# T-amairi/block-lanczos-algorithm-parallelization

Hardware: AMD Instinct MI355X
Metric: nnz*n mod-p MAC/s (higher is better)
Workload: dtype u64; 1 GPU; JGD_GL7d/GL7d19-shape synthetic: 1911130x1955309, 37322725 nnz, --prime 2^61-1 --n 8 --left; parallelism=single GPU, matrix=seeded synthetic, uniform columns (SURVEY 8(d)); real .mtx not on the box, timing=one region of 2050 steps, max over ranks per region

## Files before the change

### block-lanczos-algorithm-parallelization_amd/csrc/blz_api.hip

```cpp
#include <dlfcn.h>
#include <unistd.h>
#include <rccl/rccl.h>

#include <algorithm>
#include <cmath>
#include <cstdio>
#include <cstdlib>
#include <cstring>
#include <memory>
#include <vector>
#include <atomic>
#include <chrono>
#include <condition_variable>
#include <mutex>

#include "blz_internal.h"
#include "blz_kernels.h"
#include "blz_border.h"
#include "blz_devio.h"
#include "blz_devalg.h"
#include "blz_devsmall.h"
#include "blz_devfuse.h"
#include "blz_devrank.h"
#include "blz_devw32.h"
// ... 144 lines not shown
	u64 *small = nullptr, *partial = nullptr;
	u64 *dot_send = nullptr;
	u64 *dot_recv = nullptr;
	int max_dot_blocks = 0;
	DevCtl *ctl = nullptr;
	DevCtl host_ctl{};
	DevCtl *ctl_pinned = nullptr, *ctl_pinned_dev = nullptr;
	ncclComm_t comm = nullptr;
	blz_loop_group *loop = nullptr;
	int loop_rank = -1;
	std::vector<int32_t> perm[2], inv[2];
	bool reorder = true;
	bool pack = true;
	bool fuse_dot = true;
	bool selfdot = true;
	u64 *partial_self = nullptr;
	int max_self_blocks = 0;
	bool fuse_local_off = false;
	int un = 0;
	bool use_graph = false;
	bool explicit_p = false;
	bool p_implicit = false;
	long long rot_swaps = 0;
	hipGraphExec_t iter_graph = nullptr;
	bool external_exchange = false;
	bool force_comm = false;
	hipStream_t cstream = nullptr;
	hipEvent_t ev_snap_go = nullptr, ev_snap_done = nullptr;
	void *snap_host[2] = { nullptr, nullptr };
	void *snap_dev[2] = { nullptr, nullptr };
// ... 201 lines not shown
		c->cfg.mfma_img = nullptr;
		HIPCHK(hipMalloc(&c->cfg.mfma_img, ortho_mfma_image_bytes()));
	}
	{
		const char *npn = getenv("BLZ_NO_PANEL");
		c->cfg.panel = !(npn && npn[0] == '1');
	}
	const char *np = getenv("BLZ_NO_PACK");
	c->pack = !(np && np[0] == '1');
	const char *nr = getenv("BLZ_NO_REORDER");
	c->reorder = !(nr && nr[0] == '1');
	const char *nf = getenv("BLZ_NO_FUSE");
	c->fuse_dot = !(nf && nf[0] == '1');
	const char *nsf = getenv("BLZ_NO_SELFDOT");
	c->selfdot = !(nsf && nsf[0] == '1');
	const char *ug = getenv("BLZ_GRAPH");
	c->use_graph = ug && ug[0] == '1';
	const char *xp = getenv("BLZ_EXPLICIT_P");
	c->explicit_p = xp && xp[0] == '1';
	if (const char *ac = getenv("BLZ_AG_CHUNKS"))
		if (atoi(ac) >= 1 && atoi(ac) <= 64)
			c->ag_chunks = atoi(ac);
	HIPCHK(hipStreamCreateWithFlags(&c->stream, hipStreamNonBlocking));
	HIPCHK(hipStreamCreateWithFlags(&c->xstream, hipStreamNonBlocking));
	HIPCHK(hipEventCreateWithFlags(&c->ev_prod, hipEventDisableTiming));
	HIPCHK(hipEventCreate(&c->ev0));
	HIPCHK(hipEventCreate(&c->ev1));
	HIPCHK(hipMalloc(&c->small, small_words(np_) * sizeof(u64)));
	HIPCHK(hipMemset(c->small, 0, small_words(np_) * sizeof(u64)));
	{
		int rc_ = explicit_p_state(c);
		if (rc_ != BLZ_OK)
			return rc_;
	}
	HIPCHK(hipMalloc(&c->dot_send, (size_t)2 * np_ * np_ * sizeof(u64)));
	HIPCHK(hipMemset(c->dot_send, 0, (size_t)2 * np_ * np_ * sizeof(u64)));
	HIPCHK(hipMalloc(&c->dot_recv, (size_t)2 * np_ * np_ * sizeof(u64)));
	HIPCHK(hipMemset(c->dot_recv, 0, (size_t)2 * np_ * np_ * sizeof(u64)));
	c->max_dot_blocks = c->cfg.num_cu * (np_ <= 8 ? 16 : 8);
	HIPCHK(hipMalloc(&c->partial, (size_t)c->max_dot_blocks * 2 * np_ * np_ * sizeof(u64)));
	if (c->selfdot && np_ <= 8) {
		c->max_self_blocks = c->cfg.num_cu * std::max(8, c->cfg.spmv_blocks_per_cu) + 8;
		HIPCHK(hipMalloc(&c->partial_self, (size_t)c->max_self_blocks * np_ * np_ * sizeof(u64)));
	}
// ... 972 lines not shown
static inline bool iteration_fuses(const blz_ctx *c)
{
	return c->fuse_dot && !c->fuse_local_off && spmv_dot_supported(c->cfg) && c->count[0] > 0 && !c->short_side[c->right];
}

static inline bool selfdot_path(const blz_ctx *c)
{
	if (!c->selfdot || !c->partial_self || !c->have_matrix || !iteration_fuses(c) || exchanging(c) || c->nranks != 1 || c->bd.rhs
	    || c->use_graph || c->short_side[0] || c->short_side[1] || c->csr[0].size() != 1 || c->csr[1].size() != 1)
		return false;
	return spmv_self_ok(c->cfg, c->csr[!c->right][0], false, c->max_self_blocks)
	       && spmv_self_ok(c->cfg, c->csr[c->right][0], true, c->max_dot_blocks);
}

extern "C" int blz_selfdot_active(const blz_ctx *c) { return c && selfdot_path(c) ? 1 : 0; }

static void plan_launch(const SpmvGrids &g, blz_plan_launch *o)
{
	o->form = g.form == SPMV_FORM_PANEL ? BLZ_FORM_PANEL : (g.form == SPMV_FORM_STAGED ? BLZ_FORM_STAGED : BLZ_FORM_SPMV);
	o->xcd_ranges = g.xcd;
	o->split_log2 = g.split_log2;
	o->st_gathers = g.gathers;
	o->grid_stream = g.blocks;
	o->grid_heavy = g.hb;
	o->grid_combine = g.cb;
	o->grid_medium = g.mb;
}

extern "C" int blz_slab_plan(const blz_ctx *c, int transpose, int piece, blz_plan *out)
{
// ... 247 lines not shown
	int g = 0;
	while (g + 1 < c->nranks && c->bounds[sd][g + 1] <= r)
		g++;
	return g;
}

static int small_off(const blz_ctx *c, int which, int *words)
{
	const int nn = c->cfg.n * c->cfg.n;
	*words = which == BLZ_D ? c->cfg.n : nn;
	switch (which) {
	case BLZ_VTAV: return 0;
	case BLZ_VTAAV: return nn;
	case BLZ_WINV: return 2 * nn;
	case BLZ_D: return 3 * nn;
	default: return -1;
	}
}

extern "C" int blz_set_small(blz_ctx *c, int which, const uint64_t *host)
{
	if (!c || !host)
		return blz_fail(BLZ_EINVAL, "blz_set_small: NULL argument");
	HIPCHK(hipSetDevice(c->device));
	int words, off = small_off(c, which, &words);
	if (off < 0)
		return blz_fail(BLZ_EINVAL, "blz_set_small: unknown operand %d", which);
	HIPCHK(hipStreamSynchronize(c->stream));
	std::vector<u64> dev((size_t)words, 0);
	const int un = c->un, np = c->cfg.n;
// ... 352 lines not shown
{
	NEED_MATRIX(c);
	int rc = materialize_p(c);
	if (rc != BLZ_OK)
		return rc;
	rc = enqueue_ortho(c);
	if (rc != BLZ_OK)
		return rc;
	HIPCHK(hipStreamSynchronize(c->stream));
	return BLZ_OK;
}

static int enqueue_iteration(blz_ctx *c)
{
	int rc;
	if (selfdot_path(c)) {
		int nb1 = 0, nb2 = 0;
		{
			Span sp(c, PK_SPMV1);
			HIPCHK(launch_spmv_self(c->cfg, c->csr[!c->right][0], operand_ptr(c, BLZ_V), slab_ptr(c, BLZ_TMP), false,
						c->partial_self, c->max_self_blocks, &nb1, c->ctl, c->stream));
		}
		{
			Span sp(c, PK_SPMV2);
			HIPCHK(launch_spmv_self(c->cfg, c->csr[c->right][0], operand_ptr(c, BLZ_TMP), slab_ptr(c, BLZ_AV), true, c->partial,
						c->max_dot_blocks, &nb2, c->ctl, c->stream));
		}
		{
			Span sp(c, PK_DOT);
			HIPCHK(launch_dot_finalize_pair(c->cfg, c->partial_self, nb1, c->partial, nb2, c->small, c->ctl, c->stream));
		}
	} else if ((rc = enqueue_product(c, !c->right, BLZ_V, BLZ_TMP, false, nullptr)) != BLZ_OK) {
		return rc;
	} else if (iteration_fuses(c)) {
		int nb = 0;
		if ((rc = enqueue_product(c, c->right, BLZ_TMP, BLZ_AV, true, &nb)) != BLZ_OK) return rc;
		{
			Span sp(c, PK_DOT);
			HIPCHK(launch_dot_finalize(c->cfg, c->partial, nb, dot_out(c), c->ctl, c->stream));
		}
		if ((rc = allreduce_dots(c)) != BLZ_OK) return rc;
	} else {
		if ((rc = enqueue_product(c, c->right, BLZ_TMP, BLZ_AV, false, nullptr)) != BLZ_OK) return rc;
		if ((rc = enqueue_dot(c)) != BLZ_OK) return rc;
	}
	const bool img = ortho_uses_mfma(c->cfg, c->count[0]);
	const bool rot = img && !c->use_graph && !c->explicit_p;
	{
		Span sp(c, PK_SEMI);
		HIPCHK(launch_semi_inverse(c->cfg, dot_sums(c), c->small, c->ctl, 1, img, c->stream, rot ? c->un : 0));
	}
	if (!rot)
		return enqueue_ortho(c, img);
	const int np = c->cfg.n;
	Span sp(c, PK_ORTHO);
	if (np == 16)
		HIPCHK(launch_block_mul_gated(c->cfg, c->slab[BLZ_P], c->count[0], np, np, c->small + small_Emat(np), c->ctl,
					      c->small + small_materialize(np), c->stream));
	HIPCHK(launch_orthogonalize_rotate(c->cfg, slab_ptr(c, BLZ_V), slab_ptr(c, BLZ_AV), slab_ptr(c, BLZ_P), c->count[0],
					   c->small, c->ctl, c->stream));
	std::swap(c->slab[BLZ_V], c->slab[BLZ_P]);
	c->p_implicit = true;
	c->rot_swaps++;
	return BLZ_OK;
}
// ... 1981 lines not shown
```

### block-lanczos-algorithm-parallelization_amd/csrc/blz_kernels.h

```cpp
#ifndef BLZ_KERNELS_H
#define BLZ_KERNELS_H

#include <hip/hip_runtime.h>
#include <type_traits>
#include "modp.h"

#define HEAVY_SEG 4096u
struct HeavySeg {
	int row;
	u32 k0, k1;
	int whole_row;
};
struct HeavyRow {
	int row, first, count;
};

struct XcdRows {
	long long begin[9];
};

struct DevCsr {
	int64_t rows = 0, cols = 0, nnz = 0;
	u32 *row_ptr = nullptr;
	int *col_idx = nullptr;
// ... 80 lines not shown
SpmvGrids spmv_grids(const KernelCfg &c, const DevCsr &A, bool dot, int max_blocks);

hipError_t launch_spmv(const KernelCfg &c, const DevCsr &A, const void *X, void *Y, int accum, const DevCtl *ctl,
		       hipStream_t s);

bool spmv_dot_supported(const KernelCfg &c);
hipError_t launch_spmv_dot(const KernelCfg &c, const DevCsr &A, const void *X, void *Y, const void *Vd, int accum,
			   u64 *partial, int max_blocks, int *nblocks, const DevCtl *ctl, hipStream_t s);

hipError_t launch_block_dot(const KernelCfg &c, const void *V, const void *AV, int64_t rows, u64 *partial,
			    int max_blocks, int *nblocks, const DevCtl *ctl, hipStream_t s);
hipError_t launch_dot_finalize(const KernelCfg &c, const u64 *partial, int nblocks, u64 *out, const DevCtl *ctl,
			       hipStream_t s);

bool spmv_self_ok(const KernelCfg &c, const DevCsr &A, bool second, int max_blocks);
hipError_t launch_spmv_self(const KernelCfg &c, const DevCsr &A, const void *X, void *Y, bool second, u64 *partial,
			    int max_blocks, int *nblocks, const DevCtl *ctl, hipStream_t s);
hipError_t launch_dot_finalize_pair(const KernelCfg &c, const u64 *pa, int na, const u64 *pb, int nb, u64 *out, const DevCtl *ctl,
				    hipStream_t s);
hipError_t launch_dot_finalize_half(const KernelCfg &c, const u64 *partial, int nblocks, u64 *out, int half, const DevCtl *ctl,
				    hipStream_t s);

hipError_t launch_semi_inverse(const KernelCfg &c, const u64 *sums, u64 *small, DevCtl *ctl, int in_loop, int build_img,
			       hipStream_t s, int rot_un = 0);

hipError_t launch_orthogonalize(const KernelCfg &c, void *V, const void *AV, void *P, int64_t rows,
				const u64 *small, const DevCtl *ctl, hipStream_t s, bool img_ready = false);
bool ortho_uses_mfma(const KernelCfg &c, int64_t rows);

hipError_t launch_publish_ctl(const DevCtl *ctl, DevCtl *host_mapped, hipStream_t s);

hipError_t launch_copy(const KernelCfg &c, void *dst, const void *src, size_t bytes, hipStream_t s);

hipError_t launch_reduce_modp(const KernelCfg &c, void *dst, const void *src, int64_t words, const DevCtl *ctl, hipStream_t s);

size_t ortho_mfma_image_bytes(void);
bool ortho_mfma_supported(const KernelCfg &c);
hipError_t launch_orthogonalize_mfma(const KernelCfg &c, void *V, const void *AV, void *P, int64_t rows, const u64 *small,
				     const DevCtl *ctl, hipStream_t s, bool img_ready, bool rotate = false);
// ... 11 lines not shown

int rref_partial_blocks(const KernelCfg &c, int64_t rows, int n);
hipError_t launch_rref_partial(const KernelCfg &c, const void *X, int64_t rows, int ld, int n, u64 *stack, int *ctl,
			       hipStream_t s);
hipError_t launch_rref_merge(const KernelCfg &c, const u64 *stack, int64_t rows, const int *rows_dev, int n, u64 *E, int *info,
			     hipStream_t s);
hipError_t launch_block_mul(const KernelCfg &c, void *X, int64_t rows, int ld, int n, const u64 *Z, hipStream_t s);
hipError_t launch_block_mul_gated(const KernelCfg &c, void *X, int64_t rows, int ld, int n, const u64 *Z, const DevCtl *ctl,
				  const u64 *gate, hipStream_t s);

__host__ __device__ constexpr size_t small_E(int n) { return (size_t)6 * n * n; }
__host__ __device__ constexpr size_t small_Emat(int n) { return (size_t)7 * n * n; }
__host__ __device__ constexpr size_t small_skip_p(int n) { return (size_t)8 * n * n; }
__host__ __device__ constexpr size_t small_materialize(int n) { return (size_t)8 * n * n + 1; }
__host__ __device__ constexpr size_t small_words(int n) { return (size_t)8 * n * n + 8; }

#ifdef __cplusplus
template <typename T> struct TypeTag { using type = T; };
template <int V> using IntTag = std::integral_constant<int, V>;
template <bool V> using BoolTag = std::integral_constant<bool, V>;
#define DISPATCH_INLINE static inline __attribute__((always_inline))

template <typename F> DISPATCH_INLINE auto with_word_reducer(const KernelCfg &c, F &&f)
{
	if (c.word == 4)
		return c.mers == 31 ? f(TypeTag<u32>{}, IntTag<31>{}) : f(TypeTag<u32>{}, IntTag<0>{});
	return c.mers == 61 ? f(TypeTag<u64>{}, IntTag<61>{}) : f(TypeTag<u64>{}, IntTag<0>{});
}

template <int... Gs, typename F> DISPATCH_INLINE bool with_lane_group(int G, F &&f)
// ... 35 lines not shown
```

### block-lanczos-algorithm-parallelization_amd/csrc/blz_kernels.hip

```cpp
#include "blz_kernels.h"
#include "ortho_img.h"

#include <algorithm>
#include <atomic>
#include <type_traits>

#define BLOCK 256

MODP_DEV u64 shfl64(u64 x, int src)
{
	const u32 lo = (u32)__shfl((int)(u32)x, src, 64), hi = (u32)__shfl((int)(u32)(x >> 32), src, 64);
	return ((u64)hi << 32) | lo;
}

MODP_DEV u64 bperm64(u64 x, int src_lane_x4)
{
	const u32 lo = (u32)__builtin_amdgcn_ds_bpermute(src_lane_x4, (int)(u32)x);
	const u32 hi = (u32)__builtin_amdgcn_ds_bpermute(src_lane_x4, (int)(u32)(x >> 32));
	return ((u64)hi << 32) | lo;
}

template <bool NARROW>
MODP_DEV u64 bperm_word(u64 x, int src_lane_x4)
{
// ... 813 lines not shown
			e = (lo + per) < e ? (lo + per) : e;
		}
		Acc acc;
		acc_zero(acc);
		spmv_accumulate<W, TAILB, VM, MERS>(acc, k, e, ci, va, spal, X, n, xl, m, vh);
		for (int off = G; off < (G << split_log2); off <<= 1)
			acc_add_acc(acc, shfl_xor64(acc.lo, off), shfl_xor64(acc.hi, off));
		if (lane < n && part == 0) {
			if (accum)
				acc_add(acc, Y[(size_t)r * n + lane]);
			Y[(size_t)r * n + lane] = (W)acc_reduce<MERS>(acc, m);
		}
	}
}

template <typename W, int MERS, int NT, bool TAILB, int VM = VM_U32, bool SELF = false>
__global__ void __launch_bounds__(BLOCK)
k_spmv_dot(const u32 *__restrict__ rp, const int *__restrict__ ci, const u32 *__restrict__ va,
	   const u32 *__restrict__ vh, const u32 *__restrict__ pal, const W *__restrict__ X, W *__restrict__ Y, const W *__restrict__ Vd,
	   long long rows, int accum, u32 heavy, ModP m, u64 *__restrict__ partial, XcdRows xr,
	   const DevCtl *__restrict__ ctl)
{
	if (ctl->stop)
		return;
	using DS = DotState<typename std::conditional<sizeof(W) == 4, AccS, Acc>::type, MERS, NT, BLOCK, true, SELF>;
	__shared__ u64 red[DS::WAVES][DS::SLOTS][NT];
	__shared__ u32 spal_store[VM == VM_WIDE ? 2 * BLOCK : BLOCK];
	const u32 *spal = pal ? spal_store : nullptr;
	if (pal) {
		spal_store[threadIdx.x] = pal[threadIdx.x];
		if (VM == VM_WIDE)
			spal_store[BLOCK + threadIdx.x] = pal[BLOCK + threadIdx.x];
	}
	__syncthreads();
	const int t = threadIdx.x, lane = t & (NT - 1), gbase = (t & 63) - lane;
	long long r = ((long long)blockIdx.x * BLOCK + t) / NT;
	long long ng = (long long)gridDim.x * (BLOCK / NT);
	if (xr.begin[0] >= 0) {
		const int xcd = blockIdx.x & 7;
		r = xr.begin[xcd] + ((long long)(blockIdx.x >> 3) * BLOCK + t) / NT;
		rows = xr.begin[xcd + 1];
		ng = (long long)(gridDim.x >> 3) * (BLOCK / NT);
	}
	DS ds;
	ds.init();
	for (; r < rows; r += ng) {
		const u32 k = rp[r], e = rp[r + 1];
		if (e - k > heavy)
			continue;
		u64 vi = 0;
		if constexpr (!SELF)
			vi = Vd[(size_t)r * NT + lane];
		Acc acc;
		acc_zero(acc);
		spmv_accumulate<W, TAILB, VM, MERS>(acc, k, e, ci, va, spal, X, NT, lane, m, vh);
		if (accum)
			acc_add(acc, Y[(size_t)r * NT + lane]);
// ... 147 lines not shown
	heavy_fork(c, A, s);
	const int form = spmv_form(c, A, true);
	if (form == SPMV_FORM_PANEL)
		return panel_dispatch<W, MERS, true>(c, A, X, Y, Vd, accum, partial, max_blocks, nblocks, ctl, s);
	if (form == SPMV_FORM_STAGED)
		return staged_dispatch<W, MERS, true>(c, A, X, Y, Vd, accum, partial, max_blocks, nblocks, ctl, s);
	const SpmvGrids g = stream_dot_grids(c, A, max_blocks);
	const long long blocks = g.blocks, hb = g.hb, cb = g.cb, mb = g.mb;
	const XcdRows xr = xcd_rows(A, g.xcd);
	*nblocks = (int)(blocks + hb + cb + mb);
	const bool known = with_lane_group<1, 2, 4, 8>(c.n, [&](auto nt) {
		constexpr int N = decltype(nt)::value;
		with_value_mode<W>(A, [&](auto vm, auto tailb) {
			hipLaunchKernelGGL((k_spmv_dot<W, MERS, N, decltype(tailb)::value, decltype(vm)::value>), dim3((unsigned)blocks),
					   dim3(BLOCK), 0, s, A.row_ptr, A.col_idx, A.val, A.val_hi, A.palette, X, Y, Vd, (long long)A.rows,
					   accum, A.heavy_thr, c.m, partial, xr, ctl);
		});
		if (hb || mb)
			launch_heavy<W, N, MERS, true>(c, A, X, Y, Vd, accum, partial, (int)blocks, hb, ctl, s);
	});
	return known ? hipGetLastError() : hipErrorInvalidValue;
}

bool spmv_dot_supported(const KernelCfg &c)
{
	return c.n == 1 || c.n == 2 || c.n == 4 || c.n == 8;
}

bool spmv_self_ok(const KernelCfg &c, const DevCsr &A, bool second, int max_blocks)
{
	if (!spmv_dot_supported(c) || A.rows <= 0 || A.n_heavy || A.n_medium || A.n_multi || spmv_form(c, A, second) != SPMV_FORM_STREAM)
		return false;
	const SpmvGrids g = second ? stream_dot_grids(c, A, max_blocks) : stream_grids(c, A);
	return g.ok && g.split_log2 == 0 && g.blocks >= 1 && g.blocks <= max_blocks && !g.hb && !g.cb && !g.mb;
}

template <typename W, int MERS>
static hipError_t spmv_self_dispatch(const KernelCfg &c, const DevCsr &A, const W *X, W *Y, bool second, u64 *partial,
				     int max_blocks, int *nblocks, const DevCtl *ctl, hipStream_t s)
{
	if (!spmv_self_ok(c, A, second, max_blocks))
		return hipErrorInvalidValue;
	const SpmvGrids g = second ? stream_dot_grids(c, A, max_blocks) : stream_grids(c, A);
	const long long blocks = g.blocks;
	const XcdRows xr = xcd_rows(A, g.xcd);
	*nblocks = (int)blocks;
	const bool known = with_lane_group<1, 2, 4, 8>(c.n, [&](auto nt) {
		constexpr int N = decltype(nt)::value;
		with_value_mode<W>(A, [&](auto vm, auto tailb) {
			constexpr int VM = decltype(vm)::value;
			constexpr bool TAILB = decltype(tailb)::value;
			if (second)
				hipLaunchKernelGGL((k_spmv_dot<W, MERS, N, TAILB, VM, true>), dim3((unsigned)blocks), dim3(BLOCK), 0, s,
						   A.row_ptr, A.col_idx, A.val, A.val_hi, A.palette, X, Y, (const W *)nullptr, (long long)A.rows,
						   0, A.heavy_thr, c.m, partial, xr, ctl);
			else
				hipLaunchKernelGGL((k_spmv<W, N, MERS, TAILB, VM, true>), dim3((unsigned)blocks), dim3(BLOCK), 0, s,
						   A.row_ptr, A.col_idx, A.val, A.val_hi, A.palette, X, Y, (long long)A.rows, N, 0, 0,
						   A.heavy_thr, c.m, xr, ctl, partial);
		});
	});
	return known ? hipGetLastError() : hipErrorInvalidValue;
}

hipError_t launch_spmv_self(const KernelCfg &c, const DevCsr &A, const void *X, void *Y, bool second, u64 *partial,
			    int max_blocks, int *nblocks, const DevCtl *ctl, hipStream_t s)
{
	return with_word_reducer(c, [&](auto wt, auto mers) {
		using W = typename decltype(wt)::type;
		return spmv_self_dispatch<W, decltype(mers)::value>(c, A, (const W *)X, (W *)Y, second, partial, max_blocks, nblocks, ctl, s);
	});
}

hipError_t launch_spmv_dot(const KernelCfg &c, const DevCsr &A, const void *X, void *Y, const void *Vd, int accum,
			   u64 *partial, int max_blocks, int *nblocks, const DevCtl *ctl, hipStream_t s)
{
	return with_word_reducer(c, [&](auto wt, auto mers) {
		using W = typename decltype(wt)::type;
		return spmv_dot_dispatch<W, decltype(mers)::value>(c, A, (const W *)X, (W *)Y, (const W *)Vd, accum, partial, max_blocks,
								   nblocks, ctl, s);
	});
}



struct XcdTiles {
// ... 1153 lines not shown
				acc_zero(acc);
				acc_mac64(acc, pv, *w);
				if (!two)
					acc_set(acc, acc_reduce<MERS>(acc, m));
				acc_mac64(acc, neg, wy);
				*w = acc_reduce<MERS>(acc, m);
			}
			if (s)
				*s = mulres<MERS>(*s, pv, m);
		}
	}
	*mask = bits;
	return found;
}

template <int MERS, int LG, bool IMG>
__global__ void __launch_bounds__(IMG ? 1024 : 64)
k_semi_inverse_reg(const u64 *__restrict__ sums, u64 *__restrict__ small, DevCtl *__restrict__ ctl, int n, ModP m, int in_loop,
		   unsigned char *__restrict__ img, int rot_un)
{
	constexpr int G = 1 << LG, T = IMG ? 1024 : 64;
	const int nn = n * n, lane = threadIdx.x, i = (lane & 63) >> LG, k = lane & (G - 1);
	const bool valid = lane < 64 && i < n && k < n;
	const int e = valid ? i * n + k : 0;
	const int stop = in_loop ? ctl->stop : 0;
	const u64 xr = sums[e], yr = sums[nn + e];
	const u64 eo = (IMG && rot_un) ? small[small_E(n) + e] : 0;
	if (stop)
		return;
	__shared__ u64 coef[IMG ? 7 * 64 : 1];
	__shared__ int init_sh[IMG ? OG<8>::NE : 1];
	if (lane < 64) {
		u64 *vtAv = small, *vtAAv = small + nn, *winv = small + 2 * nn, *dvec = small + 3 * nn;
		u64 *cmat = small + 4 * nn, *vtAvd = small + 5 * nn;
		const u64 x0 = valid ? reduce128<MERS>(0, xr, m) : 0, y0 = valid ? reduce128<MERS>(0, yr, m) : 0;
		if (valid) {
			vtAv[e] = x0;
			vtAAv[e] = y0;
		}
		u64 sel = 0, dbits = 0;
		u64 a = x0, w = (valid && i == k) ? 1 : 0, s = 1;
		int npiv = ff_sweep_reg<MERS, LG>(a, &w, &s, n, m, &dbits);
		if (npiv != n) {
			a = x0;
			ff_sweep_reg<MERS, LG>(a, nullptr, nullptr, n, m, &sel);
			const bool both = valid && ((sel >> i) & 1) && ((sel >> k) & 1);
			a = both ? x0 : 0;
			w = (valid && i == k && ((sel >> i) & 1)) ? 1 : 0;
			s = 1;
			npiv = ff_sweep_reg<MERS, LG>(a, &w, &s, n, m, &dbits);
		}
		u64 q = 1;
#pragma unroll
		for (int r = 0; r < G; r++) {
			const u64 sr = readlane64(s, r << LG);
			if (r < n) {
				const u64 t = mulres<MERS>(q, sr, m);
				q = r == i ? q : t;
			}
		}
		const u64 all = readlane64(mulres<MERS>(q, s, m), 0);
		const u64 mine = mulres<MERS>(dev_invmod_any<MERS>(all, m), q, m);
		const u64 wn = valid ? mulres<MERS>(w, mine, m) : 0;
		if (valid)
			winv[e] = wn;
		if (lane < n)
			dvec[lane] = (dbits >> lane) & 1;
		const bool dk = (dbits >> k) & 1;
		const u64 sp = dk ? y0 : x0;
		Acc acc;
		acc_zero(acc);
		u32 cnt = 0;
		static_for<0, G>([&](auto qc) {
			constexpr int Q = decltype(qc)::value;
			const u64 wiq = col_bcast<Q, LG>(wn), sqk = shfl64(sp, (Q << LG) + k);
			if (Q < n) {
				acc_mac64(acc, wiq, sqk);
				if (++cnt == m.chunk) {
					cnt = 0;
					acc_set(acc, acc_reduce<MERS>(acc, m));
				}
			}
		});
		u64 ce = 0, ve = 0;
		if (valid) {
			const u64 r = acc_reduce<MERS>(acc, m);
			ce = r ? m.p - r : 0;
			ve = (dk && x0) ? m.p - x0 : 0;
			cmat[e] = ce;
			vtAvd[e] = ve;
		}
		u64 fe = ve, ge = 0;
		if (IMG && rot_un && npiv > 0) {
			const u64 want = (1ull << rot_un) - 1;
			acc_zero(acc);
			cnt = 0;
			static_for<0, G>([&](auto qc) {
				constexpr int Q = decltype(qc)::value;
				const u64 eiq = col_bcast<Q, LG>(eo), vqk = shfl64(ve, (Q << LG) + k);
				acc_mac64(acc, eiq, vqk);
				if (++cnt == m.chunk) {
					cnt = 0;
					acc_set(acc, acc_reduce<MERS>(acc, m));
				}
			});
			fe = acc_reduce<MERS>(acc, m);
			const bool full = (dbits & want) == want;
			ge = (full || dk) ? 0 : eo;
			small[small_E(n) + e] = full ? wn : (i == k ? 1 : 0);
			if (lane == 0)
				small[small_skip_p(n)] = full ? 1 : 0;
		}
		if (IMG) {
			coef[2 * 64 + lane] = wn;
			coef[4 * 64 + lane] = ce;
			coef[5 * 64 + lane] = fe;
			coef[6 * 64 + lane] = ge;
		}
		if (lane == 0) {
			ctl->npiv = npiv;
			if (in_loop) {
				if (npiv == 0)
					ctl->stop = 1;
				else
					ctl->iterations += 1;
			}
		}
	}
	if constexpr (IMG) {
		__syncthreads();
		ortho_image_build<8>(coef, img, init_sh, lane, T, rot_un != 0);
	}
}

hipError_t launch_semi_inverse(const KernelCfg &c, const u64 *sums, u64 *small, DevCtl *ctl, int in_loop, int build_img,
			       hipStream_t s, int rot_un)
{
	if (rot_un && !(in_loop && build_img && rot_un <= c.n))
		return hipErrorInvalidValue;
	int G = 1, LG = 0;
	while (G < c.n) {
		G <<= 1;
		LG++;
	}
	unsigned char *img = (unsigned char *)c.mfma_img;
	if (build_img && !(ortho_mfma_supported(c) && img))
		return hipErrorInvalidValue;
// ... 708 lines not shown
```

### block-lanczos-algorithm-parallelization_amd/python/blz.py

```python
import ctypes as C
import os

import numpy as np

PKG = os.path.dirname(os.path.dirname(os.path.abspath(__file__)))
LIB_PATH = os.path.join(PKG, "lib", "libblz_hip.so")

V, TMP, AV, P = 0, 1, 2, 3
VTAV, VTAAV, WINV, D = 0, 1, 2, 3
OK, EINVAL, EIO, EFORMAT, ENOMEM, EHIP, ENOGPU, ECOMM = 0, -1, -2, -3, -4, -5, -6, -7

U64P = C.POINTER(C.c_uint64)
_lib = None


class BlzError(RuntimeError):
    def __init__(self, code, msg):
        super().__init__(f"blz error {code}: {msg}")
        self.code = code


class Coo(C.Structure):
    _fields_ = [("nrows", C.c_int64), ("ncols", C.c_int64), ("nnz", C.c_int64),
                ("i", C.POINTER(C.c_int32)), ("j", C.POINTER(C.c_int32)), ("x", C.POINTER(C.c_uint32))]
# ... 1198 lines not shown
        done, stopped, ms = C.c_int(0), C.c_int(0), C.c_float(0)
        check(lib().blz_iterate(self.h, C.c_int(max_iters), C.byref(done), C.byref(stopped), C.byref(ms)))
        return int(done.value), bool(stopped.value), float(ms.value)

    @property
    def iterations(self):
        return int(lib().blz_iterations(self.h))

    @property
    def p_implicit(self):
        return int(lib().blz_p_implicit(self.h))

    @property
    def selfdot_active(self):
        return int(lib().blz_selfdot_active(self.h))

    def set_iterations(self, its):
        check(lib().blz_set_iterations(self.h, C.c_int64(its)))

    def final_check(self):
        a, b = C.c_int(0), C.c_int(0)
        check(lib().blz_final_check(self.h, C.byref(a), C.byref(b)))
        return bool(a.value), bool(b.value)

    def block_rref(self, block):
        E = np.zeros(self.n * self.n, dtype=np.uint64)
        rank = C.c_int(0)
        piv = np.zeros(self.n, dtype=np.int32)
        check(lib().blz_block_rref(self.h, C.c_int(block), ptr(E), C.byref(rank),
                                   piv.ctypes.data_as(C.POINTER(C.c_int32))))
# ... 118 lines not shown
```

### include/blz.h

```cpp
#ifndef BLZ_H
#define BLZ_H

#include <stddef.h>
#include <stdint.h>

#ifdef __cplusplus
extern "C" {
#endif

#define BLZ_OK          0
#define BLZ_EINVAL     -1
#define BLZ_EIO        -2
#define BLZ_EFORMAT    -3
#define BLZ_ENOMEM     -4
#define BLZ_EHIP       -5
#define BLZ_ENOGPU     -6
#define BLZ_ECOMM      -7

#define BLZ_MAX_N      64
#define BLZ_MAX_RHS    16

enum { BLZ_V = 0, BLZ_TMP = 1, BLZ_AV = 2, BLZ_P = 3 };
enum { BLZ_VTAV = 0, BLZ_VTAAV = 1, BLZ_WINV = 2, BLZ_D = 3 };

typedef struct blz_ctx blz_ctx;

const char *blz_last_error(void);
int blz_version(void);


typedef struct {
	int64_t nrows, ncols, nnz;
	int32_t *i, *j;
	uint32_t *x;
} blz_coo;

typedef struct {
	int64_t rows, cols, nnz;
// ... 242 lines not shown
			      const uint64_t *const *a0, const uint64_t *const *a1, uint32_t *z0, int64_t ldz0, uint32_t *z1,
			      int64_t ldz1, void *stream);

int blz_spmv(blz_ctx *ctx, int transpose, int src_block, int dst_block);

int blz_block_dot(blz_ctx *ctx, uint64_t *vtAv, uint64_t *vtAAv);

int blz_semi_inverse(blz_ctx *ctx, int *npiv, uint64_t *winv, uint64_t *d);

int blz_orthogonalize(blz_ctx *ctx);

int blz_iterate(blz_ctx *ctx, int max_iters, int *done, int *stopped, float *ms);
int64_t blz_iterations(const blz_ctx *ctx);
int blz_p_implicit(const blz_ctx *ctx);
int blz_selfdot_active(const blz_ctx *ctx);
int blz_set_iterations(blz_ctx *ctx, int64_t iterations);

int blz_final_check(blz_ctx *ctx, int *v_nonzero, int *vtm_zero);

int blz_block_rref(blz_ctx *ctx, int block, uint64_t *rref, int *rank, int32_t *pivots);

int blz_kernel_basis(blz_ctx *ctx, int *k, uint64_t *z);

int blz_solution(blz_ctx *ctx, uint64_t *x, int *status);

int blz_solution_block(blz_ctx *ctx, uint64_t *x, int *status);

int blz_snapshot_begin(blz_ctx *c);
int blz_snapshot_wait(blz_ctx *c, uint64_t *v, uint64_t *p, int64_t *iterations);

// ... 25 lines not shown
```

Baseline: 418.7 billion MAC/s.

## Overlap V^T A V semi-inverse with second SpMV via extra workgroup

Adds one extra workgroup to the second self-dot SpMV launch. It reduces the first SpMV's V^T A V partials and runs the pivoting and inverse part of the semi-inverse while the SpMV streams. The later semi-inverse kernel then only finishes the C matrix from V^T A^2 V, and the dot finalize handles a single half. This moves the serial small-matrix inverse off the critical path. In exchange it costs an occupancy check to make sure the extra block is co-resident, extra scratch words in the small buffer, and more kernel variants.

New measurement: 422.4 billion MAC/s, median of 6. About the same (+0.9%).

```diff
diff --git a/block-lanczos-algorithm-parallelization_amd/csrc/blz_api.hip b/block-lanczos-algorithm-parallelization_amd/csrc/blz_api.hip
--- a/block-lanczos-algorithm-parallelization_amd/csrc/blz_api.hip
+++ b/block-lanczos-algorithm-parallelization_amd/csrc/blz_api.hip
@@ -182,6 +182,10 @@
 	bool pack = true;
 	bool fuse_dot = true;
 	bool selfdot = true;
+	bool early_inverse = true;
+	const void *early_slab = nullptr;
+	long long early_rows = -1;
+	bool early_resident = false;
 	u64 *partial_self = nullptr;
 	int max_self_blocks = 0;
 	bool fuse_local_off = false;
@@ -413,6 +417,8 @@
 	c->fuse_dot = !(nf && nf[0] == '1');
 	const char *nsf = getenv("BLZ_NO_SELFDOT");
 	c->selfdot = !(nsf && nsf[0] == '1');
+	const char *nei = getenv("BLZ_NO_EARLY_INVERSE");
+	c->early_inverse = !(nei && nei[0] == '1');
 	const char *ug = getenv("BLZ_GRAPH");
 	c->use_graph = ug && ug[0] == '1';
 	const char *xp = getenv("BLZ_EXPLICIT_P");
@@ -425,8 +431,8 @@
 	HIPCHK(hipEventCreateWithFlags(&c->ev_prod, hipEventDisableTiming));
 	HIPCHK(hipEventCreate(&c->ev0));
 	HIPCHK(hipEventCreate(&c->ev1));
-	HIPCHK(hipMalloc(&c->small, small_words(np_) * sizeof(u64)));
-	HIPCHK(hipMemset(c->small, 0, small_words(np_) * sizeof(u64)));
+	HIPCHK(hipMalloc(&c->small, small_alloc_words(np_) * sizeof(u64)));
+	HIPCHK(hipMemset(c->small, 0, small_alloc_words(np_) * sizeof(u64)));
 	{
 		int rc_ = explicit_p_state(c);
 		if (rc_ != BLZ_OK)
@@ -1429,6 +1435,21 @@
 }
 
 extern "C" int blz_selfdot_active(const blz_ctx *c) { return c && selfdot_path(c) ? 1 : 0; }
+
+static inline bool early_path(blz_ctx *c)
+{
+	if (!c->early_inverse || !selfdot_path(c) || c->cfg.n > 8)
+		return false;
+	const DevCsr &A = c->csr[c->right][0];
+	if (c->early_slab != (const void *)A.row_ptr || c->early_rows != (long long)A.rows) {
+		c->early_slab = (const void *)A.row_ptr;
+		c->early_rows = (long long)A.rows;
+		c->early_resident = spmv_self_early_resident(c->cfg, A, c->max_dot_blocks);
+	}
+	return c->early_resident;
+}
+
+extern "C" int blz_early_inverse_active(blz_ctx *c) { return c && early_path(c) ? 1 : 0; }
 
 static void plan_launch(const SpmvGrids &g, blz_plan_launch *o)
 {
@@ -1706,6 +1727,8 @@
 	case BLZ_VTAAV: return nn;
 	case BLZ_WINV: return 2 * nn;
 	case BLZ_D: return 3 * nn;
+	case BLZ_C: return 4 * nn;
+	case BLZ_VTAVD: return 5 * nn;
 	default: return -1;
 	}
 }
@@ -2088,7 +2111,10 @@
 static int enqueue_iteration(blz_ctx *c)
 {
 	int rc;
-	if (selfdot_path(c)) {
+	const bool img = ortho_uses_mfma(c->cfg, c->count[0]);
+	const bool rot = img && !c->use_graph && !c->explicit_p;
+	const bool early = early_path(c);
+	if (early || selfdot_path(c)) {
 		int nb1 = 0, nb2 = 0;
 		{
 			Span sp(c, PK_SPMV1);
@@ -2097,12 +2123,23 @@
 		}
 		{
 			Span sp(c, PK_SPMV2);
+			EarlyInverse ea;
+			if (early) {
+				ea.rows = c->partial_self;
+				ea.nrows = nb1;
+				ea.small = c->small;
+				ea.rot_un = rot ? c->un : 0;
+			}
 			HIPCHK(launch_spmv_self(c->cfg, c->csr[c->right][0], operand_ptr(c, BLZ_TMP), slab_ptr(c, BLZ_AV), true, c->partial,
-						c->max_dot_blocks, &nb2, c->ctl, c->stream));
+						c->max_dot_blocks, &nb2, c->ctl, c->stream, ea));
 		}
 		{
 			Span sp(c, PK_DOT);
-			HIPCHK(launch_dot_finalize_pair(c->cfg, c->partial_self, nb1, c->partial, nb2, c->small, c->ctl, c->stream));
+			if (early) {
+				HIPCHK(launch_dot_finalize_half(c->cfg, c->partial, nb2, c->small, 1, c->ctl, c->stream));
+			} else {
+				HIPCHK(launch_dot_finalize_pair(c->cfg, c->partial_self, nb1, c->partial, nb2, c->small, c->ctl, c->stream));
+			}
 		}
 	} else if ((rc = enqueue_product(c, !c->right, BLZ_V, BLZ_TMP, false, nullptr)) != BLZ_OK) {
 		return rc;
@@ -2118,11 +2155,13 @@
 		if ((rc = enqueue_product(c, c->right, BLZ_TMP, BLZ_AV, false, nullptr)) != BLZ_OK) return rc;
 		if ((rc = enqueue_dot(c)) != BLZ_OK) return rc;
 	}
-	const bool img = ortho_uses_mfma(c->cfg, c->count[0]);
-	const bool rot = img && !c->use_graph && !c->explicit_p;
 	{
 		Span sp(c, PK_SEMI);
-		HIPCHK(launch_semi_inverse(c->cfg, dot_sums(c), c->small, c->ctl, 1, img, c->stream, rot ? c->un : 0));
+		if (early) {
+			HIPCHK(launch_semi_late(c->cfg, c->small + (size_t)c->cfg.n * c->cfg.n, c->small, c->ctl, img, c->stream, rot ? c->un : 0));
+		} else {
+			HIPCHK(launch_semi_inverse(c->cfg, dot_sums(c), c->small, c->ctl, 1, img, c->stream, rot ? c->un : 0));
+		}
 	}
 	if (!rot)
 		return enqueue_ortho(c, img);
diff --git a/block-lanczos-algorithm-parallelization_amd/csrc/blz_kernels.h b/block-lanczos-algorithm-parallelization_amd/csrc/blz_kernels.h
--- a/block-lanczos-algorithm-parallelization_amd/csrc/blz_kernels.h
+++ b/block-lanczos-algorithm-parallelization_amd/csrc/blz_kernels.h
@@ -118,8 +118,15 @@
 			       hipStream_t s);
 
 bool spmv_self_ok(const KernelCfg &c, const DevCsr &A, bool second, int max_blocks);
+struct EarlyInverse {
+	const u64 *rows = nullptr;
+	int nrows = 0;
+	u64 *small = nullptr;
+	int rot_un = 0;
+};
 hipError_t launch_spmv_self(const KernelCfg &c, const DevCsr &A, const void *X, void *Y, bool second, u64 *partial,
-			    int max_blocks, int *nblocks, const DevCtl *ctl, hipStream_t s);
+			    int max_blocks, int *nblocks, const DevCtl *ctl, hipStream_t s, const EarlyInverse &early = EarlyInverse());
+bool spmv_self_early_resident(const KernelCfg &c, const DevCsr &A, int max_blocks);
 hipError_t launch_dot_finalize_pair(const KernelCfg &c, const u64 *pa, int na, const u64 *pb, int nb, u64 *out, const DevCtl *ctl,
 				    hipStream_t s);
 hipError_t launch_dot_finalize_half(const KernelCfg &c, const u64 *partial, int nblocks, u64 *out, int half, const DevCtl *ctl,
@@ -127,6 +134,9 @@
 
 hipError_t launch_semi_inverse(const KernelCfg &c, const u64 *sums, u64 *small, DevCtl *ctl, int in_loop, int build_img,
 			       hipStream_t s, int rot_un = 0);
+
+hipError_t launch_semi_late(const KernelCfg &c, const u64 *sums, u64 *small, DevCtl *ctl, int build_img, hipStream_t s,
+			    int rot_un = 0);
 
 hipError_t launch_orthogonalize(const KernelCfg &c, void *V, const void *AV, void *P, int64_t rows,
 				const u64 *small, const DevCtl *ctl, hipStream_t s, bool img_ready = false);
@@ -168,6 +178,8 @@
 __host__ __device__ constexpr size_t small_skip_p(int n) { return (size_t)8 * n * n; }
 __host__ __device__ constexpr size_t small_materialize(int n) { return (size_t)8 * n * n + 1; }
 __host__ __device__ constexpr size_t small_words(int n) { return (size_t)8 * n * n + 8; }
+__host__ __device__ constexpr size_t small_early(int n) { return small_words(n); }
+__host__ __device__ constexpr size_t small_alloc_words(int n) { return small_early(n) + (size_t)6 * n * n + 8; }
 
 #ifdef __cplusplus
 template <typename T> struct TypeTag { using type = T; };
diff --git a/block-lanczos-algorithm-parallelization_amd/csrc/blz_kernels.hip b/block-lanczos-algorithm-parallelization_amd/csrc/blz_kernels.hip
--- a/block-lanczos-algorithm-parallelization_amd/csrc/blz_kernels.hip
+++ b/block-lanczos-algorithm-parallelization_amd/csrc/blz_kernels.hip
@@ -851,17 +851,31 @@
 	}
 }
 
-template <typename W, int MERS, int NT, bool TAILB, int VM = VM_U32, bool SELF = false>
+template <int MERS, int NT, bool ROT>
+MODP_DEV void spmv_early_inverse(const u64 *__restrict__ rows, int nrows, u64 *__restrict__ small, const ModP &m, int rot_un,
+				 u64 (*part)[NT * NT]);
+
+template <typename W, int MERS, int NT, bool TAILB, int VM = VM_U32, bool SELF = false, bool EARLY = false>
 __global__ void __launch_bounds__(BLOCK)
 k_spmv_dot(const u32 *__restrict__ rp, const int *__restrict__ ci, const u32 *__restrict__ va,
 	   const u32 *__restrict__ vh, const u32 *__restrict__ pal, const W *__restrict__ X, W *__restrict__ Y, const W *__restrict__ Vd,
 	   long long rows, int accum, u32 heavy, ModP m, u64 *__restrict__ partial, XcdRows xr,
-	   const DevCtl *__restrict__ ctl)
+	   const DevCtl *__restrict__ ctl, EarlyInverse early)
 {
 	if (ctl->stop)
 		return;
 	using DS = DotState<typename std::conditional<sizeof(W) == 4, AccS, Acc>::type, MERS, NT, BLOCK, true, SELF>;
 	__shared__ u64 red[DS::WAVES][DS::SLOTS][NT];
+	static_assert(SELF || !EARLY, "the extra workgroup rides on the self form");
+	const unsigned nwg = gridDim.x - (EARLY ? 1u : 0u);
+	if constexpr (EARLY) {
+		__shared__ u64 early_part[BLOCK / 64 - 1][NT * NT];
+		if (blockIdx.x == nwg) {
+			spmv_early_inverse<MERS, NT, NT == 8 && MERS == 61 && sizeof(W) == 8>(early.rows, early.nrows, early.small, m,
+											      early.rot_un, early_part);
+			return;
+		}
+	}
 	__shared__ u32 spal_store[VM == VM_WIDE ? 2 * BLOCK : BLOCK];
 	const u32 *spal = pal ? spal_store : nullptr;
 	if (pal) {
@@ -872,12 +886,12 @@
 	__syncthreads();
 	const int t = threadIdx.x, lane = t & (NT - 1), gbase = (t & 63) - lane;
 	long long r = ((long long)blockIdx.x * BLOCK + t) / NT;
-	long long ng = (long long)gridDim.x * (BLOCK / NT);
+	long long ng = (long long)nwg * (BLOCK / NT);
 	if (xr.begin[0] >= 0) {
 		const int xcd = blockIdx.x & 7;
 		r = xr.begin[xcd] + ((long long)(blockIdx.x >> 3) * BLOCK + t) / NT;
 		rows = xr.begin[xcd + 1];
-		ng = (long long)(gridDim.x >> 3) * (BLOCK / NT);
+		ng = (long long)(nwg >> 3) * (BLOCK / NT);
 	}
 	DS ds;
 	ds.init();
@@ -1055,7 +1069,7 @@
 		with_value_mode<W>(A, [&](auto vm, auto tailb) {
 			hipLaunchKernelGGL((k_spmv_dot<W, MERS, N, decltype(tailb)::value, decltype(vm)::value>), dim3((unsigned)blocks),
 					   dim3(BLOCK), 0, s, A.row_ptr, A.col_idx, A.val, A.val_hi, A.palette, X, Y, Vd, (long long)A.rows,
-					   accum, A.heavy_thr, c.m, partial, xr, ctl);
+					   accum, A.heavy_thr, c.m, partial, xr, ctl, EarlyInverse());
 		});
 		if (hb || mb)
 			launch_heavy<W, N, MERS, true>(c, A, X, Y, Vd, accum, partial, (int)blocks, hb, ctl, s);
@@ -1078,9 +1092,10 @@
 
 template <typename W, int MERS>
 static hipError_t spmv_self_dispatch(const KernelCfg &c, const DevCsr &A, const W *X, W *Y, bool second, u64 *partial,
-				     int max_blocks, int *nblocks, const DevCtl *ctl, hipStream_t s)
-{
-	if (!spmv_self_ok(c, A, second, max_blocks))
+				     int max_blocks, int *nblocks, const DevCtl *ctl, hipStream_t s, const EarlyInverse &early,
+				     long long *resident = nullptr)
+{
+	if (!spmv_self_ok(c, A, second, max_blocks) || ((early.rows || resident) && !second))
 		return hipErrorInvalidValue;
 	const SpmvGrids g = second ? stream_dot_grids(c, A, max_blocks) : stream_grids(c, A);
 	const long long blocks = g.blocks;
@@ -1091,10 +1106,20 @@
 		with_value_mode<W>(A, [&](auto vm, auto tailb) {
 			constexpr int VM = decltype(vm)::value;
 			constexpr bool TAILB = decltype(tailb)::value;
-			if (second)
+			if (resident) {
+				int per_cu = 0;
+				if (hipOccupancyMaxActiveBlocksPerMultiprocessor(&per_cu, k_spmv_dot<W, MERS, N, TAILB, VM, true, true>, BLOCK, 0)
+				    != hipSuccess)
+					per_cu = 0;
+				*resident = (long long)per_cu * c.num_cu;
+			} else if (second && early.rows)
+				hipLaunchKernelGGL((k_spmv_dot<W, MERS, N, TAILB, VM, true, true>), dim3((unsigned)blocks + 1u), dim3(BLOCK), 0, s,
+						   A.row_ptr, A.col_idx, A.val, A.val_hi, A.palette, X, Y, (const W *)nullptr, (long long)A.rows,
+						   0, A.heavy_thr, c.m, partial, xr, ctl, early);
+			else if (second)
 				hipLaunchKernelGGL((k_spmv_dot<W, MERS, N, TAILB, VM, true>), dim3((unsigned)blocks), dim3(BLOCK), 0, s,
 						   A.row_ptr, A.col_idx, A.val, A.val_hi, A.palette, X, Y, (const W *)nullptr, (long long)A.rows,
-						   0, A.heavy_thr, c.m, partial, xr, ctl);
+						   0, A.heavy_thr, c.m, partial, xr, ctl, EarlyInverse());
 			else
 				hipLaunchKernelGGL((k_spmv<W, N, MERS, TAILB, VM, true>), dim3((unsigned)blocks), dim3(BLOCK), 0, s,
 						   A.row_ptr, A.col_idx, A.val, A.val_hi, A.palette, X, Y, (long long)A.rows, N, 0, 0,
@@ -1105,12 +1130,25 @@
 }
 
 hipError_t launch_spmv_self(const KernelCfg &c, const DevCsr &A, const void *X, void *Y, bool second, u64 *partial,
-			    int max_blocks, int *nblocks, const DevCtl *ctl, hipStream_t s)
+			    int max_blocks, int *nblocks, const DevCtl *ctl, hipStream_t s, const EarlyInverse &early)
 {
 	return with_word_reducer(c, [&](auto wt, auto mers) {
 		using W = typename decltype(wt)::type;
-		return spmv_self_dispatch<W, decltype(mers)::value>(c, A, (const W *)X, (W *)Y, second, partial, max_blocks, nblocks, ctl, s);
+		return spmv_self_dispatch<W, decltype(mers)::value>(c, A, (const W *)X, (W *)Y, second, partial, max_blocks, nblocks, ctl, s,
+								    early);
 	});
+}
+
+bool spmv_self_early_resident(const KernelCfg &c, const DevCsr &A, int max_blocks)
+{
+	int nb = 0;
+	long long resident = 0;
+	const hipError_t e = with_word_reducer(c, [&](auto wt, auto mers) {
+		using W = typename decltype(wt)::type;
+		return spmv_self_dispatch<W, decltype(mers)::value>(c, A, (const W *)nullptr, (W *)nullptr, true, nullptr, max_blocks, &nb,
+								    nullptr, nullptr, EarlyInverse(), &resident);
+	});
+	return e == hipSuccess && nb + 1 <= resident;
 }
 
 hipError_t launch_spmv_dot(const KernelCfg &c, const DevCsr &A, const void *X, void *Y, const void *Vd, int accum,
@@ -2294,6 +2332,144 @@
 	return found;
 }
 
+struct SemiEarly {
+	u64 x0, wn, ve, fe, ge, en;
+	u64 dbits;
+	int npiv, full;
+};
+
+template <int MERS, int LG, bool ROT>
+MODP_DEV void semi_early_reg(u64 x0, u64 eo, int n, const ModP &m, int rot_un, SemiEarly &o)
+{
+	constexpr int G = 1 << LG;
+	const int lane = threadIdx.x, i = lane >> LG, k = lane & (G - 1);
+	const bool valid = i < n && k < n;
+	u64 sel = 0, dbits = 0;
+	u64 a = x0, w = (valid && i == k) ? 1 : 0, s = 1;
+	int npiv = ff_sweep_reg<MERS, LG>(a, &w, &s, n, m, &dbits);
+	if (npiv != n) {
+		a = x0;
+		ff_sweep_reg<MERS, LG>(a, nullptr, nullptr, n, m, &sel);
+		const bool both = valid && ((sel >> i) & 1) && ((sel >> k) & 1);
+		a = both ? x0 : 0;
+		w = (valid && i == k && ((sel >> i) & 1)) ? 1 : 0;
+		s = 1;
+		npiv = ff_sweep_reg<MERS, LG>(a, &w, &s, n, m, &dbits);
+	}
+	u64 q = 1;
+#pragma unroll
+	for (int r = 0; r < G; r++) {
+		const u64 sr = readlane64(s, r << LG);
+		if (r < n) {
+			const u64 t = mulres<MERS>(q, sr, m);
+			q = r == i ? q : t;
+		}
+	}
+	const u64 all = readlane64(mulres<MERS>(q, s, m), 0);
+	const u64 mine = mulres<MERS>(dev_invmod_any<MERS>(all, m), q, m);
+	const u64 wn = valid ? mulres<MERS>(w, mine, m) : 0;
+	const bool dk = (dbits >> k) & 1;
+	const u64 ve = (valid && dk && x0) ? m.p - x0 : 0;
+	u64 fe = ve, ge = 0, en = 0;
+	int full = 0;
+	if (ROT && rot_un && npiv > 0) {
+		const u64 want = (1ull << rot_un) - 1;
+		Acc acc;
+		acc_zero(acc);
+		u32 cnt = 0;
+		static_for<0, G>([&](auto qc) {
+			constexpr int Q = decltype(qc)::value;
+			const u64 eiq = col_bcast<Q, LG>(eo), vqk = shfl64(ve, (Q << LG) + k);
+			acc_mac64(acc, eiq, vqk);
+			if (++cnt == m.chunk) {
+				cnt = 0;
+				acc_set(acc, acc_reduce<MERS>(acc, m));
+			}
+		});
+		fe = acc_reduce<MERS>(acc, m);
+		full = (dbits & want) == want;
+		ge = (full || dk) ? 0 : eo;
+		en = full ? wn : (i == k ? 1 : 0);
+	}
+	o.x0 = x0;
+	o.wn = wn;
+	o.ve = ve;
+	o.fe = fe;
+	o.ge = ge;
+	o.en = en;
+	o.dbits = dbits;
+	o.npiv = npiv;
+	o.full = full;
+}
+
+template <int MERS, int LG>
+MODP_DEV u64 semi_late_c(const SemiEarly &ea, u64 y0, int n, const ModP &m)
+{
+	constexpr int G = 1 << LG;
+	const int lane = threadIdx.x, i = lane >> LG, k = lane & (G - 1);
+	const bool dk = (ea.dbits >> k) & 1;
+	const u64 sp = dk ? y0 : ea.x0;
+	Acc acc;
+	acc_zero(acc);
+	u32 cnt = 0;
+	static_for<0, G>([&](auto qc) {
+		constexpr int Q = decltype(qc)::value;
+		const u64 wiq = col_bcast<Q, LG>(ea.wn), sqk = shfl64(sp, (Q << LG) + k);
+		if (Q < n) {
+			acc_mac64(acc, wiq, sqk);
+			if (++cnt == m.chunk) {
+				cnt = 0;
+				acc_set(acc, acc_reduce<MERS>(acc, m));
+			}
+		}
+	});
+	if (!(i < n && k < n))
+		return 0;
+	const u64 r = acc_reduce<MERS>(acc, m);
+	return r ? m.p - r : 0;
+}
+
+template <int LG, bool IMG>
+MODP_DEV void semi_publish(const SemiEarly &ea, u64 y0, u64 ce, u64 *__restrict__ small, DevCtl *__restrict__ ctl, u64 *coef,
+			   int n, int in_loop, int rot_un)
+{
+	constexpr int G = 1 << LG;
+	const int nn = n * n, lane = threadIdx.x, i = lane >> LG, k = lane & (G - 1);
+	const bool valid = i < n && k < n;
+	const int e = valid ? i * n + k : 0;
+	u64 *vtAv = small, *vtAAv = small + nn, *winv = small + 2 * nn, *dvec = small + 3 * nn;
+	u64 *cmat = small + 4 * nn, *vtAvd = small + 5 * nn;
+	if (valid) {
+		vtAv[e] = ea.x0;
+		vtAAv[e] = y0;
+		winv[e] = ea.wn;
+		cmat[e] = ce;
+		vtAvd[e] = ea.ve;
+	}
+	if (lane < n)
+		dvec[lane] = (ea.dbits >> lane) & 1;
+	if (IMG && rot_un && ea.npiv > 0) {
+		small[small_E(n) + e] = ea.en;
+		if (lane == 0)
+			small[small_skip_p(n)] = ea.full ? 1 : 0;
+	}
+	if (IMG) {
+		coef[2 * 64 + lane] = ea.wn;
+		coef[4 * 64 + lane] = ce;
+		coef[5 * 64 + lane] = ea.fe;
+		coef[6 * 64 + lane] = ea.ge;
+	}
+	if (lane == 0) {
+		ctl->npiv = ea.npiv;
+		if (in_loop) {
+			if (ea.npiv == 0)
+				ctl->stop = 1;
+			else
+				ctl->iterations += 1;
+		}
+	}
+}
+
 template <int MERS, int LG, bool IMG>
 __global__ void __launch_bounds__(IMG ? 1024 : 64)
 k_semi_inverse_reg(const u64 *__restrict__ sums, u64 *__restrict__ small, DevCtl *__restrict__ ctl, int n, ModP m, int in_loop,
@@ -2311,106 +2487,131 @@
 	__shared__ u64 coef[IMG ? 7 * 64 : 1];
 	__shared__ int init_sh[IMG ? OG<8>::NE : 1];
 	if (lane < 64) {
-		u64 *vtAv = small, *vtAAv = small + nn, *winv = small + 2 * nn, *dvec = small + 3 * nn;
-		u64 *cmat = small + 4 * nn, *vtAvd = small + 5 * nn;
 		const u64 x0 = valid ? reduce128<MERS>(0, xr, m) : 0, y0 = valid ? reduce128<MERS>(0, yr, m) : 0;
-		if (valid) {
-			vtAv[e] = x0;
-			vtAAv[e] = y0;
-		}
-		u64 sel = 0, dbits = 0;
-		u64 a = x0, w = (valid && i == k) ? 1 : 0, s = 1;
-		int npiv = ff_sweep_reg<MERS, LG>(a, &w, &s, n, m, &dbits);
-		if (npiv != n) {
-			a = x0;
-			ff_sweep_reg<MERS, LG>(a, nullptr, nullptr, n, m, &sel);
-			const bool both = valid && ((sel >> i) & 1) && ((sel >> k) & 1);
-			a = both ? x0 : 0;
-			w = (valid && i == k && ((sel >> i) & 1)) ? 1 : 0;
-			s = 1;
-			npiv = ff_sweep_reg<MERS, LG>(a, &w, &s, n, m, &dbits);
-		}
-		u64 q = 1;
-#pragma unroll
-		for (int r = 0; r < G; r++) {
-			const u64 sr = readlane64(s, r << LG);
-			if (r < n) {
-				const u64 t = mulres<MERS>(q, sr, m);
-				q = r == i ? q : t;
-			}
-		}
-		const u64 all = readlane64(mulres<MERS>(q, s, m), 0);
-		const u64 mine = mulres<MERS>(dev_invmod_any<MERS>(all, m), q, m);
-		const u64 wn = valid ? mulres<MERS>(w, mine, m) : 0;
-		if (valid)
-			winv[e] = wn;
-		if (lane < n)
-			dvec[lane] = (dbits >> lane) & 1;
-		const bool dk = (dbits >> k) & 1;
-		const u64 sp = dk ? y0 : x0;
-		Acc acc;
-		acc_zero(acc);
-		u32 cnt = 0;
-		static_for<0, G>([&](auto qc) {
-			constexpr int Q = decltype(qc)::value;
-			const u64 wiq = col_bcast<Q, LG>(wn), sqk = shfl64(sp, (Q << LG) + k);
-			if (Q < n) {
-				acc_mac64(acc, wiq, sqk);
-				if (++cnt == m.chunk) {
-					cnt = 0;
-					acc_set(acc, acc_reduce<MERS>(acc, m));
-				}
-			}
-		});
-		u64 ce = 0, ve = 0;
-		if (valid) {
-			const u64 r = acc_reduce<MERS>(acc, m);
-			ce = r ? m.p - r : 0;
-			ve = (dk && x0) ? m.p - x0 : 0;
-			cmat[e] = ce;
-			vtAvd[e] = ve;
-		}
-		u64 fe = ve, ge = 0;
-		if (IMG && rot_un && npiv > 0) {
-			const u64 want = (1ull << rot_un) - 1;
-			acc_zero(acc);
-			cnt = 0;
-			static_for<0, G>([&](auto qc) {
-				constexpr int Q = decltype(qc)::value;
-				const u64 eiq = col_bcast<Q, LG>(eo), vqk = shfl64(ve, (Q << LG) + k);
-				acc_mac64(acc, eiq, vqk);
-				if (++cnt == m.chunk) {
-					cnt = 0;
-					acc_set(acc, acc_reduce<MERS>(acc, m));
-				}
-			});
-			fe = acc_reduce<MERS>(acc, m);
-			const bool full = (dbits & want) == want;
-			ge = (full || dk) ? 0 : eo;
-			small[small_E(n) + e] = full ? wn : (i == k ? 1 : 0);
-			if (lane == 0)
-				small[small_skip_p(n)] = full ? 1 : 0;
-		}
-		if (IMG) {
-			coef[2 * 64 + lane] = wn;
-			coef[4 * 64 + lane] = ce;
-			coef[5 * 64 + lane] = fe;
-			coef[6 * 64 + lane] = ge;
-		}
-		if (lane == 0) {
-			ctl->npiv = npiv;
-			if (in_loop) {
-				if (npiv == 0)
-					ctl->stop = 1;
-				else
-					ctl->iterations += 1;
-			}
-		}
+		SemiEarly ea;
+		semi_early_reg<MERS, LG, IMG>(x0, eo, n, m, rot_un, ea);
+		const u64 ce = semi_late_c<MERS, LG>(ea, y0, n, m);
+		semi_publish<LG, IMG>(ea, y0, ce, small, ctl, coef, n, in_loop, rot_un);
 	}
 	if constexpr (IMG) {
 		__syncthreads();
 		ortho_image_build<8>(coef, img, init_sh, lane, T, rot_un != 0);
 	}
+}
+
+enum { EARLY_X = 0, EARLY_W, EARLY_V, EARLY_F, EARLY_G, EARLY_E, EARLY_PANELS };
+enum { EARLY_DBITS = 0, EARLY_NPIV, EARLY_FULL };
+
+template <int MERS, int NT, bool ROT>
+MODP_DEV void spmv_early_inverse(const u64 *__restrict__ rows, int nrows, u64 *__restrict__ small, const ModP &m, int rot_un,
+				 u64 (*part)[NT * NT])
+{
+	constexpr int NN = NT * NT, LG = NT == 8 ? 3 : (NT == 4 ? 2 : (NT == 2 ? 1 : 0)), RL = BLOCK / NN;
+	const int t = threadIdx.x, lane = t & 63, wave = t >> 6, e = t & (NN - 1);
+	const u64 eo = (ROT && rot_un && t < 64) ? small[small_E(NT) + e] : 0;
+	u64 s = 0;
+	int b = t / NN;
+	for (; b + 7 * RL < nrows; b += 8 * RL) {
+		u64 x[8];
+#pragma unroll
+		for (int q = 0; q < 8; q++)
+			x[q] = rows[(size_t)(b + q * RL) * NN + e];
+#pragma unroll
+		for (int q = 0; q < 8; q++)
+			s = addmod(s, x[q], m.p);
+	}
+	for (; b < nrows; b += RL)
+		s = addmod(s, rows[(size_t)b * NN + e], m.p);
+#pragma unroll
+	for (int off = NN; off < 64; off <<= 1)
+		s = addmod(s, shfl_xor64(s, off), m.p);
+	if (wave > 0 && lane < NN)
+		part[wave - 1][lane] = s;
+	__syncthreads();
+	if (wave != 0)
+		return;
+	const bool valid = lane < NN;
+#pragma unroll
+	for (int w = 0; w < BLOCK / 64 - 1; w++)
+		s = addmod(s, part[w][e], m.p);
+	SemiEarly ea;
+	semi_early_reg<MERS, LG, ROT>(valid ? s : 0, eo, NT, m, rot_un, ea);
+	u64 *ep = small + small_early(NT);
+	if (valid) {
+		ep[EARLY_X * NN + e] = ea.x0;
+		ep[EARLY_W * NN + e] = ea.wn;
+		ep[EARLY_V * NN + e] = ea.ve;
+		ep[EARLY_F * NN + e] = ea.fe;
+		ep[EARLY_G * NN + e] = ea.ge;
+		ep[EARLY_E * NN + e] = ea.en;
+	}
+	if (lane == 0) {
+		ep[EARLY_PANELS * NN + EARLY_DBITS] = ea.dbits;
+		ep[EARLY_PANELS * NN + EARLY_NPIV] = (u64)ea.npiv;
+		ep[EARLY_PANELS * NN + EARLY_FULL] = (u64)ea.full;
+	}
+}
+
+template <int MERS, int LG, bool IMG>
+__global__ void __launch_bounds__(IMG ? 1024 : 64)
+k_semi_late(const u64 *__restrict__ sums, u64 *__restrict__ small, DevCtl *__restrict__ ctl, ModP m, unsigned char *__restrict__ img,
+	    int rot_un)
+{
+	constexpr int G = 1 << LG, NN = G * G, T = IMG ? 1024 : 64;
+	const int lane = threadIdx.x;
+	const bool valid = lane < NN;
+	const int e = valid ? lane : 0;
+	const u64 *ep = small + small_early(G);
+	const int stop = ctl->stop;
+	const u64 yr = sums[e];
+	SemiEarly ea;
+	ea.x0 = ep[EARLY_X * NN + e];
+	ea.wn = ep[EARLY_W * NN + e];
+	ea.ve = ep[EARLY_V * NN + e];
+	ea.fe = ep[EARLY_F * NN + e];
+	ea.ge = ep[EARLY_G * NN + e];
+	ea.en = ep[EARLY_E * NN + e];
+	ea.dbits = ep[EARLY_PANELS * NN + EARLY_DBITS];
+	ea.npiv = (int)ep[EARLY_PANELS * NN + EARLY_NPIV];
+	ea.full = (int)ep[EARLY_PANELS * NN + EARLY_FULL];
+	if (stop)
+		return;
+	__shared__ u64 coef[IMG ? 7 * 64 : 1];
+	__shared__ int init_sh[IMG ? OG<8>::NE : 1];
+	if (lane < 64) {
+		if (!valid)
+			ea.x0 = ea.wn = ea.ve = ea.fe = ea.ge = ea.en = 0;
+		const u64 y0 = valid ? yr : 0;
+		const u64 ce = semi_late_c<MERS, LG>(ea, y0, G, m);
+		semi_publish<LG, IMG>(ea, y0, ce, small, ctl, coef, G, 1, rot_un);
+	}
+	if constexpr (IMG) {
+		__syncthreads();
+		ortho_image_build<8>(coef, img, init_sh, lane, T, rot_un != 0);
+	}
+}
+
+hipError_t launch_semi_late(const KernelCfg &c, const u64 *sums, u64 *small, DevCtl *ctl, int build_img, hipStream_t s, int rot_un)
+{
+	if (!spmv_dot_supported(c) || (rot_un && !(build_img && rot_un <= c.n)))
+		return hipErrorInvalidValue;
+	unsigned char *img = (unsigned char *)c.mfma_img;
+	if (build_img && !(ortho_mfma_supported(c) && img && c.n == 8))
+		return hipErrorInvalidValue;
+	if (build_img) {
+		hipLaunchKernelGGL((k_semi_late<61, 3, true>), dim3(1), dim3(1024), 0, s, sums, small, ctl, c.m, img, rot_un);
+		return hipGetLastError();
+	}
+	const bool known = with_lane_group<1, 2, 4, 8>(c.n, [&](auto nt) {
+		constexpr int N = decltype(nt)::value, LG = N == 8 ? 3 : (N == 4 ? 2 : (N == 2 ? 1 : 0));
+		if (c.mers == 61)
+			hipLaunchKernelGGL((k_semi_late<61, LG, false>), dim3(1), dim3(64), 0, s, sums, small, ctl, c.m, img, 0);
+		else if (c.mers == 31)
+			hipLaunchKernelGGL((k_semi_late<31, LG, false>), dim3(1), dim3(64), 0, s, sums, small, ctl, c.m, img, 0);
+		else
+			hipLaunchKernelGGL((k_semi_late<0, LG, false>), dim3(1), dim3(64), 0, s, sums, small, ctl, c.m, img, 0);
+	});
+	return known ? hipGetLastError() : hipErrorInvalidValue;
 }
 
 hipError_t launch_semi_inverse(const KernelCfg &c, const u64 *sums, u64 *small, DevCtl *ctl, int in_loop, int build_img,
diff --git a/block-lanczos-algorithm-parallelization_amd/python/blz.py b/block-lanczos-algorithm-parallelization_amd/python/blz.py
--- a/block-lanczos-algorithm-parallelization_amd/python/blz.py
+++ b/block-lanczos-algorithm-parallelization_amd/python/blz.py
@@ -7,7 +7,7 @@
 LIB_PATH = os.path.join(PKG, "lib", "libblz_hip.so")
 
 V, TMP, AV, P = 0, 1, 2, 3
-VTAV, VTAAV, WINV, D = 0, 1, 2, 3
+VTAV, VTAAV, WINV, D, CMAT, VTAVD = 0, 1, 2, 3, 4, 5
 OK, EINVAL, EIO, EFORMAT, ENOMEM, EHIP, ENOGPU, ECOMM = 0, -1, -2, -3, -4, -5, -6, -7
 
 U64P = C.POINTER(C.c_uint64)
@@ -1236,6 +1236,10 @@
     @property
     def selfdot_active(self):
         return int(lib().blz_selfdot_active(self.h))
+
+    @property
+    def early_inverse_active(self):
+        return int(lib().blz_early_inverse_active(self.h))
 
     def set_iterations(self, its):
         check(lib().blz_set_iterations(self.h, C.c_int64(its)))
diff --git a/include/blz.h b/include/blz.h
--- a/include/blz.h
+++ b/include/blz.h
@@ -21,7 +21,7 @@
 #define BLZ_MAX_RHS    16
 
 enum { BLZ_V = 0, BLZ_TMP = 1, BLZ_AV = 2, BLZ_P = 3 };
-enum { BLZ_VTAV = 0, BLZ_VTAAV = 1, BLZ_WINV = 2, BLZ_D = 3 };
+enum { BLZ_VTAV = 0, BLZ_VTAAV = 1, BLZ_WINV = 2, BLZ_D = 3, BLZ_C = 4, BLZ_VTAVD = 5 };
 
 typedef struct blz_ctx blz_ctx;
 
@@ -294,6 +294,7 @@
 int64_t blz_iterations(const blz_ctx *ctx);
 int blz_p_implicit(const blz_ctx *ctx);
 int blz_selfdot_active(const blz_ctx *ctx);
+int blz_early_inverse_active(blz_ctx *ctx);
 int blz_set_iterations(blz_ctx *ctx, int64_t iterations);
 
 int blz_final_check(blz_ctx *ctx, int *v_nonzero, int *vtm_zero);
```
